# lixirui142/VidToMe

Measured on AMD Instinct MI355X. Metric: denoising steps/sec, 16-frame 512x512 SD-1.5 chunk, ratio=0.5, higher is better.
Workload: dtype f16 tokens; matching f16-MFMA filter + f32 exact refine (f32-identical indices); attention f16 MFMA with f32 accumulate

## Files before the change

### vidtome_amd/csrc/match_filter.hip

```cpp
#include "common.h"
#include "ablate.h"

#include <cstdlib>

#include <algorithm>
#include <type_traits>

namespace {

constexpr int FBD = 128;
constexpr int FBS = 256;
constexpr int FBK = 64;
constexpr int THREADS = 256;
constexpr int CAP = 64;
constexpr float SCALE = 1024.0f;
constexpr float INV_S2 = 1.0f / (1024.0f * 1024.0f);
#ifndef VTM_FILTER_PRODUCTS
#define VTM_FILTER_PRODUCTS 1
#endif
constexpr bool SRC_LO = VTM_FILTER_PRODUCTS >= 3;
constexpr bool DST_LO = VTM_FILTER_PRODUCTS >= 2;
static_assert(DST_LO || !SRC_LO, "the src lo half is only used together with the dst lo half");
constexpr float WINDOW = SRC_LO ? 6.5e-4f : DST_LO ? 1.5e-3f : 2.4e-3f;
constexpr int MAX_C = 1280;

typedef float f32x16 __attribute__((ext_vector_type(16)));
typedef _Float16 h16x8 __attribute__((ext_vector_type(8)));
typedef uint32_t u32x4 __attribute__((ext_vector_type(4)));
typedef __attribute__((address_space(3))) void lds_void;
typedef const __attribute__((address_space(1))) void glb_void;

using vtm::to_f32;

template <typename T>
__device__ __forceinline__ const T *pool_row(const T *x0, int64_t P0, const T *x1, int64_t P1, int64_t b,
                                             int64_t r, int64_t C) {
    return r < P0 ? x0 + (b * P0 + r) * C : x1 + (b * P1 + (r - P0)) * C;
}

template <typename T>
__device__ __forceinline__ void load8(const T *src, float (&f)[8]) {
    if constexpr (sizeof(T) == 4) {
        const float4 v0 = *reinterpret_cast<const float4 *>(src);
        const float4 v1 = *reinterpret_cast<const float4 *>(src + 4);
        f[0] = v0.x; f[1] = v0.y; f[2] = v0.z; f[3] = v0.w;
        f[4] = v1.x; f[5] = v1.y; f[6] = v1.z; f[7] = v1.w;
    } else {
        const uint4 v = *reinterpret_cast<const uint4 *>(src);
        const T *e = reinterpret_cast<const T *>(&v);
#pragma unroll
        for (int j = 0; j < 8; ++j) f[j] = to_f32(e[j]);
    }
}

__device__ __forceinline__ float vmax3(float a, float b, float c) {
    float d;
    asm("v_max3_f32 %0, %1, %2, %3" : "=v"(d) : "v"(a), "v"(b), "v"(c));
    return d;
}
__device__ __forceinline__ float vmax2(float a, float b) {
    float d;
    asm("v_max_f32 %0, %1, %2" : "=v"(d) : "v"(a), "v"(b));
    return d;
}

struct RowDivisor {
    float n, r1, lo;
};
__device__ __forceinline__ RowDivisor row_divisor(float n) {
    const float r = __builtin_amdgcn_rcpf(n);
    const float e = __builtin_fmaf(-n, r, 1.0f);
    return {n, __builtin_fmaf(e, r, r), fmaxf(0x1p-102f, n * 0x1p-124f)};
}
__device__ __forceinline__ bool div_ok(float x, const RowDivisor &d) { return __builtin_fabsf(x) >= d.lo || x == 0.0f; }
__device__ __forceinline__ float div_by_row(float x, const RowDivisor &d) {
    const float q = x * d.r1;
    const float t = __builtin_fmaf(-d.n, q, x);
    const float q1 = __builtin_fmaf(t, d.r1, q);
    const float t2 = __builtin_fmaf(-d.n, q1, x);
    return __builtin_fmaf(t2, d.r1, q1);
}

__device__ __forceinline__ uint32_t orderable(float f) {
    if (f != f) return 0xffffffffu;
    const uint32_t u = __float_as_uint(f + 0.0f);
    return (u & 0x80000000u) ? ~u : (u | 0x80000000u);
}
__device__ __forceinline__ float from_orderable(uint32_t o) {
    if (o == 0u) return -INFINITY;
    return __uint_as_float((o & 0x80000000u) ? (o & 0x7fffffffu) : ~o);
}

struct SplitArgs {
    const int32_t *rows;
    int64_t n;
    float *norms;
    uint4 *out_hi, *out_lo;
    int64_t n_pad;
    float *rest, *tile_rest;
    float *rest2, *tile_rest2;
};

#ifndef VTM_PREP_PIECES
#define VTM_PREP_PIECES 10
#endif
#ifndef VTM_PREP_WAVES
#define VTM_PREP_WAVES 4
#endif
constexpr int PREP_WAVES = VTM_PREP_WAVES;
constexpr int PREP_PIECES = VTM_PREP_PIECES;
constexpr int PREP_STRIDE = PREP_PIECES * 16 + 16;

template <typename T>
__global__ __launch_bounds__(64 * PREP_WAVES) void prep_operand(const T *__restrict__ x0, int64_t P0,
                                                    const T *__restrict__ x1, int64_t P1, int64_t B, int64_t C,
                                                    SplitArgs A0, SplitArgs A1, int64_t C_pad,
                                                    uint32_t *__restrict__ zero, int64_t zero_words,
                                                    unsigned long long *__restrict__ best, int64_t nbest, int64_t cut,
                                                    int64_t cut2) {
    static_assert(sizeof(T) == 2 || sizeof(T) == 4, "element size");
    static_assert(PREP_WAVES % 2 == 0, "a 128-row tile is two waves of one workgroup");
    __shared__ float wave_rest[PREP_WAVES], wave_rest2[PREP_WAVES];
    constexpr int EPP = 16 / (int)sizeof(T);
    __shared__ __attribute__((aligned(16))) char slab[PREP_WAVES][64 * PREP_STRIDE];
    const int64_t G = C_pad / 8;
    const int64_t gid = (int64_t)blockIdx.x * blockDim.x + threadIdx.x, gsz = (int64_t)gridDim.x * blockDim.x;
    for (int64_t w = gid; w < zero_words; w += gsz) zero[w] = 0u;
    for (int64_t w = gid; w < nbest; w += gsz) best[w] = 0ull;
    const int lane = threadIdx.x & 63, wave = threadIdx.x >> 6;
    char *my = slab[wave];

    int64_t idx = gid;
    const bool second = idx >= B * A0.n_pad;
    if (second) idx -= B * A0.n_pad;
    const SplitArgs &A = second ? A1 : A0;
    const int64_t n = A.n, n_pad = A.n_pad;
    const bool in_range = idx < B * n_pad;
    const int64_t i = in_range ? idx % n_pad : 0, b = in_range ? idx / n_pad : 0;
    const bool real = in_range && i < n;
    const T *src = real ? pool_row(x0, P0, x1, P1, b, A.rows[b * n + i], C) : x0;

    const int pieces = (int)(C * sizeof(T) / 16);
    const int nchunks = (pieces + PREP_PIECES - 1) / PREP_PIECES;
    uint4 stage[PREP_PIECES];
    auto issue = [&](int chunk) {
#pragma unroll
        for (int t = 0; t < PREP_PIECES; ++t) {
            const int q = lane + 64 * t, r = q / PREP_PIECES, col = q % PREP_PIECES;
            const T *rp = reinterpret_cast<const T *>(__shfl((unsigned long long)reinterpret_cast<uintptr_t>(src), r, 64));
            const int piece = chunk * PREP_PIECES + col;
            stage[t] = piece < pieces ? *reinterpret_cast<const uint4 *>(rp + (int64_t)piece * EPP) : make_uint4(0, 0, 0, 0);
        }
    };
    auto to_lds = [&]() {
#pragma unroll
        for (int t = 0; t < PREP_PIECES; ++t) {
            const int q = lane + 64 * t, r = q / PREP_PIECES, col = q % PREP_PIECES;
            *reinterpret_cast<uint4 *>(my + r * PREP_STRIDE + col * 16) = stage[t];
        }
    };
    auto my_piece = [&](int col, float (&f)[EPP]) {
        const uint4 v = *reinterpret_cast<const uint4 *>(my + lane * PREP_STRIDE + col * 16);
        const T *e = reinterpret_cast<const T *>(&v);
#pragma unroll
        for (int k = 0; k < EPP; ++k) f[k] = to_f32(e[k]);
    };

    float acc = 0.0f;
    issue(0);
    for (int c = 0; c < nchunks; ++c) {
        to_lds();
        if (c + 1 < nchunks) issue(c + 1);
        const int valid = min(PREP_PIECES, pieces - c * PREP_PIECES);
        for (int col = 0; col < valid; ++col) {
            float f[EPP];
            my_piece(col, f);
#pragma unroll
            for (int k = 0; k < EPP; ++k) acc = __builtin_fmaf(f[k], f[k], acc);
        }
    }
    const float nrm = __builtin_sqrtf(acc);
    if (real) A.norms[b * n + i] = nrm;

    const float rscale = SCALE * __builtin_amdgcn_rcpf(nrm);
    uint4 *__restrict__ out_hi = in_range ? A.out_hi + (b * G) * n_pad + i : nullptr;
    uint4 *__restrict__ out_lo = (in_range && A.out_lo) ? A.out_lo + (b * G) * n_pad + i : nullptr;
    constexpr int PPG = 8 / EPP;
    float rest = 0.0f, rest2 = 0.0f;
    issue(0);
    for (int c = 0; c < nchunks; ++c) {
        to_lds();
        if (c + 1 < nchunks) issue(c + 1);
        const int valid = min(PREP_PIECES, pieces - c * PREP_PIECES);
        for (int col = 0; col + PPG <= valid; col += PPG) {
            float f[8];
            if constexpr (PPG == 1) {
                my_piece(col, f);
            } else {
                float f0[EPP], f1[EPP];
                my_piece(col, f0);
                my_piece(col + 1, f1);
#pragma unroll
                for (int k = 0; k < EPP; ++k) { f[k] = f0[k]; f[EPP + k] = f1[k]; }
            }
            uint4 vh, vl;
            _Float16 *ph = reinterpret_cast<_Float16 *>(&vh), *pl = reinterpret_cast<_Float16 *>(&vl);
#pragma unroll
            for (int e = 0; e < 8; ++e) {
                const float sc = DST_LO ? (f[e] / nrm) * SCALE : f[e] * rscale;
                const _Float16 h = (_Float16)sc;
                ph[e] = h;
                pl[e] = (_Float16)(sc - (float)h);
            }
            if (!real) vh = vl = make_uint4(0, 0, 0, 0);
            const int64_t g = ((int64_t)c * PREP_PIECES + col) / PPG;
            if (g * 8 >= cut2) {
                float sq = 0.0f;
#pragma unroll
                for (int e = 0; e < 8; ++e) sq = __builtin_fmaf((float)ph[e], (float)ph[e], sq);
                rest2 += sq;
                if (g * 8 >= cut) rest += sq;
            }
            if (in_range) {
                out_hi[g * n_pad] = vh;
                if (out_lo) out_lo[g * n_pad] = vl;
            }
        }
    }
    if (in_range)
        for (int64_t g = C / 8; g < G; ++g) {
            out_hi[g * n_pad] = make_uint4(0, 0, 0, 0);
            if (out_lo) out_lo[g * n_pad] = make_uint4(0, 0, 0, 0);
        }
    const bool bad_row = real && !(nrm >= 0x1p-100f && nrm <= 0x1p100f);
    const float rnorm = !real ? 0.0f : bad_row ? INFINITY : __builtin_sqrtf(rest) * (1.0f + 0x1p-16f);
    if (in_range && A.rest) A.rest[b * n_pad + i] = rnorm;
    float wm = rnorm;
#pragma unroll
    for (int off = 32; off > 0; off >>= 1) wm = fmaxf(wm, __shfl_xor(wm, off, 64));
    if (lane == 0) wave_rest[wave] = wm;
    const float rnorm2 = !real ? 0.0f : bad_row ? INFINITY : __builtin_sqrtf(rest2) * (1.0f + 0x1p-16f);
    if (in_range && A.rest2) A.rest2[b * n_pad + i] = rnorm2;
    float wm2 = rnorm2;
#pragma unroll
    for (int off = 32; off > 0; off >>= 1) wm2 = fmaxf(wm2, __shfl_xor(wm2, off, 64));
    if (lane == 0) wave_rest2[wave] = wm2;
    __syncthreads();
    if (in_range && A.tile_rest && (threadIdx.x & 127) == 0)
        A.tile_rest[(b * n_pad + i) / 128] = fmaxf(wave_rest[wave], wave_rest[wave + 1]);
    if (in_range && A.tile_rest2 && (threadIdx.x & 127) == 0)
        A.tile_rest2[(b * n_pad + i) / 128] = fmaxf(wave_rest2[wave], wave_rest2[wave + 1]);
}

template <bool SCOUT>
__global__ __launch_bounds__(THREADS, 2) void filter_kernel(
    const uint4 *__restrict__ ah, const uint4 *__restrict__ al, const uint4 *__restrict__ bh,
    const uint4 *__restrict__ bl, int64_t Ns, int64_t Nd, int64_t Ns_pad, int64_t Nd_pad, int64_t C_pad, int align,
    int ns_tiles, int nd_tiles, int nsplit, int tiles_per_split, int total_src_tiles, int patch_tiles,
    unsigned int *__restrict__ amax, int *__restrict__ cnt, uint2 *__restrict__ cand, int cand_rows, int *__restrict__ flags,
    const float *__restrict__ rest_a, const float *__restrict__ rest_bt, int KP, int count_blocks,
    unsigned int *__restrict__ tilemap, int map_words) {
    __shared__ __attribute__((aligned(16))) uint4 sA[2][DST_LO ? 2 : 1][8 * FBD];

    const int tid = threadIdx.x, lane = tid & 63;
    const int wave = __builtin_amdgcn_readfirstlane(tid >> 6);
    const int l31 = lane & 31, kh = lane >> 5;

    const int xcd = blockIdx.x & 7, slot = blockIdx.x >> 3;
    const int per_group = patch_tiles * nsplit;
    const int grp = (slot / per_group) * 8 + xcd;
    const int q = slot % per_group;
    const int stg = grp * patch_tiles + q % patch_tiles;
    const int split = q / patch_tiles;
    if (stg >= total_src_tiles) return;
    const int st_ = stg % ns_tiles;
    const int bi = stg / ns_tiles;
    int jt0 = split * tiles_per_split;
    int jt1 = min(jt0 + tiles_per_split, nd_tiles);
    if (jt0 >= jt1) return;
    if constexpr (!SCOUT) {
        if (tilemap != nullptr) {
            const unsigned int *row = tilemap + (int64_t)stg * map_words;
            int lo = jt1, hi = jt0;
            for (int w = jt0 >> 5; w <= (jt1 - 1) >> 5; ++w) {
                unsigned int bits = row[w];
                if (w == (jt0 >> 5)) bits &= 0xffffffffu << (jt0 & 31);
                if (w == ((jt1 - 1) >> 5) && (jt1 & 31)) bits &= 0xffffffffu >> (32 - (jt1 & 31));
                if (bits) {
                    lo = min(lo, w * 32 + __ffs(bits) - 1);
                    hi = max(hi, w * 32 + 32 - __clz(bits));
                }
            }
            lo = __builtin_amdgcn_readfirstlane(lo);
            hi = __builtin_amdgcn_readfirstlane(hi);
            if (lo >= hi) return;
            jt0 = lo;
            jt1 = hi;
        }
    }

    const int KT = SCOUT ? KP : (int)(C_pad / FBK);
    const int64_t G = C_pad / 8;
    const int steps = (jt1 - jt0) * KT;
    int n_tested = 0, n_alive = 0;
    const uint4 *srch = ah + (int64_t)bi * G * Ns_pad, *srcl = al + (int64_t)bi * G * Ns_pad;
    const uint4 *dsth = bh + (int64_t)bi * G * Nd_pad, *dstl = bl + (int64_t)bi * G * Nd_pad;
    const int64_t srow0 = (int64_t)st_ * FBS + wave * 64;

    constexpr int NB = SRC_LO ? 4 : 2;
    const uint32_t voff_b = (uint32_t)(kh * Ns_pad + srow0 + l31) * 16u;
    const int64_t bgroup = 2 * Ns_pad;
    u32x4 rb[4][2][2];
    [[maybe_unused]] auto load_b = [&](int kt, int ks, u32x4 (&dst)[2][2]) {
        const uint4 *ph = srch + (int64_t)ABL_STREAMED(kt * 4 + ks, ks) * bgroup;
        asm volatile("global_load_dwordx4 %0, %1, %2" : "=v"(dst[0][0]) : "v"(voff_b), "s"(ph));
        asm volatile("global_load_dwordx4 %0, %1, %2 offset:512" : "=v"(dst[1][0]) : "v"(voff_b), "s"(ph));
        if constexpr (SRC_LO) {
            const uint4 *pl = srcl + (int64_t)(kt * 4 + ks) * bgroup;
            asm volatile("global_load_dwordx4 %0, %1, %2" : "=v"(dst[0][1]) : "v"(voff_b), "s"(pl));
            asm volatile("global_load_dwordx4 %0, %1, %2 offset:512" : "=v"(dst[1][1]) : "v"(voff_b), "s"(pl));
        }
    };
    auto await_b = [&](auto count_tag, u32x4 (&r)[2][2]) {
        constexpr int N = decltype(count_tag)::value;
        if constexpr (SRC_LO)
            asm volatile("s_waitcnt vmcnt(%4)" : "+v"(r[0][0]), "+v"(r[1][0]), "+v"(r[0][1]), "+v"(r[1][1]) : "n"(N));
        else
            asm volatile("s_waitcnt vmcnt(%2)" : "+v"(r[0][0]), "+v"(r[1][0]) : "n"(N));
    };
    constexpr int NPIECE = DST_LO ? 8 : 4, PG = NPIECE / 2;
    const uint4 *abase[NPIECE];
    uint32_t alds[NPIECE];
#pragma unroll
    for (int t = 0; t < NPIECE; ++t) {
// ... 275 lines not shown
            h16x8 (&fh)[4] = fa[s & 1];
            h16x8 (&fn)[4] = fa[(s + 1) & 1];
#pragma unroll
            for (int j = 0; j < 8; ++j) {
                const int sb = j >> 2, ib = j & 3;
                bool alive = true;
                if constexpr (!FIRST) alive = (live & (1u << j)) != 0u;
                if (alive) {
                    f32x16 c = acc[ib][sb];
                    if constexpr (FIRST) {
#pragma unroll
                        for (int r = 0; r < 16; ++r) c[r] = 0.0f;
                    }
                    acc[ib][sb] = __builtin_amdgcn_mfma_f32_32x32x16_f16(fh[ib], __builtin_bit_cast(h16x8, rb[s][sb][0]), c, 0, 0, 0);
                }
                __builtin_amdgcn_sched_barrier(0);
                if (j < 4) {
                    ABL_LDSREAD(if constexpr (s < 3) fn[j] = __builtin_bit_cast(h16x8, sA[buf][0][((s + 1) * 2 + kh) * FBD + j * 32 + l31]);
                                else fn[j] = __builtin_bit_cast(h16x8, sA[buf ^ 1][0][kh * FBD + j * 32 + l31]);)
                    ABL_NO_LDSREAD(fn[j] = fh[j];)
                } else if (j < 6) {
                    ABL_BLOAD(if constexpr (s < 2) load_b1(pb, s + 2, j - 4, rb[s + 2][j - 4][0]);
                              else load_b1(pbn, s - 2, j - 4, rb[s - 2][j - 4][0]);)
                } else {
                    ABL_DMA(if constexpr (s == 0) load_a_piece(pa1, buf ^ 1, j - 4);
                            if constexpr (s == 3) load_a_piece(pa2, buf, j - 6);)
                    if constexpr (s == 1)
                        asm volatile("global_load_dword %0, %1, %2 sc1" : "=v"(am[j - 6]) : "v"(voff_m[j - 6]), "s"(amax_rows));
                }
                __builtin_amdgcn_sched_barrier(0);
            }
        };
        await_b(std::integral_constant<int, ABL_AWAIT_COUNT(NB + PG)>{}, rb[0]);
        if (kt == 0) group(std::integral_constant<int, 0>{}, std::true_type{});
        else group(std::integral_constant<int, 0>{}, std::false_type{});
        group(std::integral_constant<int, 1>{}, std::false_type{});
        group(std::integral_constant<int, 2>{}, std::false_type{});
        ABL_BARRIER(asm volatile("s_waitcnt vmcnt(%0) lgkmcnt(0)" ::"n"(2 * NB + 2) : "memory"); __syncthreads();)
        group(std::integral_constant<int, 3>{}, std::false_type{});
        if (kt + 1 == KP) {
            live = prune_check(jt);
            n_tested += 8;
            n_alive += __popc(live);
            if constexpr (SCOUT) {
                if (live && lane == 0) atomicOr(&tilemap[(int64_t)stg * map_words + (jt >> 5)], 1u << (jt & 31));
            }
        }
        if constexpr (!SCOUT) {
            if (ABL_WRAP_COND(wrap && live)) collect_tile(jt, std::true_type{});
        }
        if (wrap) {
            ++jt;
            live = 0xffu;
        }
        kt = kt1;
        pb = pbn;
        pa1 = pa2;
    }
#endif
    asm volatile("s_waitcnt vmcnt(0)" ::: "memory");
    if (count_blocks && lane == 0 && n_tested) {
        if (!SCOUT && tilemap != nullptr) {
            atomicAdd(&flags[7], n_tested);
        } else {
            atomicAdd(&flags[4], n_tested);
            atomicAdd(&flags[5], n_alive);
        }
    }
    if constexpr (SCOUT) return;

#pragma unroll
    for (int sb = 0; sb < 2; ++sb) {
        const int64_t srow = srow0 + sb * 32 + l31;
        if (srow >= Ns) continue;
        float rm = runmax[sb];
        if (rm > -INFINITY) {
            const uint32_t mine = orderable(rm * INV_S2);
            const uint32_t prev = atomicMax(&amax[out_row0 + srow], mine);
            rm = fmaxf(rm, from_orderable(prev) * (SCALE * SCALE));
        }
#pragma unroll
        for (int e = 0; e < 4; ++e)
            if (cv[sb][e] >= rm - WS && cv[sb][e] > -INFINITY) push(srow, cv[sb][e], ci[sb][e]);
    }
}

template <typename T>
__global__ __launch_bounds__(256) void seed_kernel(const T *__restrict__ x0, int64_t P0, const T *__restrict__ x1, int64_t P1,
                                                   int64_t B, int64_t C, const int32_t *__restrict__ a_rows, int64_t Ns,
                                                   const int32_t *__restrict__ b_rows, int64_t Nd,
                                                   const float *__restrict__ na, const float *__restrict__ nb, int align,
                                                   int64_t seed_L, int64_t N, const int32_t *__restrict__ pos1,
                                                   const int32_t *__restrict__ table, unsigned int *__restrict__ amax, int dry,
                                                   unsigned int *__restrict__ seed_lb, float lb_margin) {
    constexpr int LPR = 8;
    const int64_t g = ((int64_t)blockIdx.x * blockDim.x + threadIdx.x) / LPR;
    const int sub = threadIdx.x & (LPR - 1);
    if (g >= B * Ns) return;
    const int64_t b = g / Ns, i = g % Ns;
    const int32_t ra = a_rows[b * Ns + i];
    int64_t pos = -1;
    if (ra < seed_L) pos = ra % N;
    else if (pos1 != nullptr && ra - P0 >= 0 && ra - P0 < P1) pos = pos1[b * P1 + (ra - P0)];
    int64_t j = -1;
    if (pos >= 0 && pos < N) j = table ? (int64_t)table[b * N + pos] : pos;
    if (j < 0 || j >= Nd) return;
    const T *pa = pool_row(x0, P0, x1, P1, b, ra, C);
    const T *pb = pool_row(x0, P0, x1, P1, b, b_rows[b * Nd + j], C);
    float acc = 0.0f;
    for (int64_t k = sub * 8; k < C; k += LPR * 8) {
        float fa[8], fb[8];
        load8(pa + k, fa);
        load8(pb + k, fb);
#pragma unroll
        for (int e = 0; e < 8; ++e) acc = __builtin_fmaf(fa[e], fb[e], acc);
    }
#pragma unroll
    for (int off = LPR / 2; off > 0; off >>= 1) acc += __shfl_xor(acc, off, 64);
    if (sub == 0) {
        const float s0 = (acc / na[b * Ns + i]) / nb[b * Nd + j];
        const float s = s0 - 1e-4f;
        const bool acc_ok = __builtin_fabsf(acc) >= 0x1p-100f || (na[b * Ns + i] >= 0x1p-40f && nb[b * Nd + j] >= 0x1p-40f);
        if (s == s && __builtin_fabsf(s) <= 1.5f && acc_ok && !dry) {
            atomicMax(&amax[align ? i : b * Ns + i], orderable(s));
            atomicMax(&seed_lb[align ? i : b * Ns + i], orderable(s0 - lb_margin));
        }
    }
}

#ifndef VTM_RROWS
#define VTM_RROWS 64
#endif
constexpr int RROWS = VTM_RROWS;
static_assert(RROWS == 32 || RROWS == 64 || RROWS == 128 || RROWS == 256, "refine rows per workgroup");
template <typename T>
__global__ __launch_bounds__(256) void refine_kernel(const T *__restrict__ x0, int64_t P0, const T *__restrict__ x1,
                                                     int64_t P1, int64_t B, int64_t C,
                                                     const int32_t *__restrict__ a_rows, int64_t Ns,
                                                     const int32_t *__restrict__ b_rows, int64_t Nd,
                                                     const float *__restrict__ na, const float *__restrict__ nb,
                                                     int align, int *__restrict__ flags, int64_t rows_out,
                                                     const unsigned int *__restrict__ amax, const int *__restrict__ cnt,
                                                     const uint2 *__restrict__ cand, int *__restrict__ ovf_cnt,
                                                     int *__restrict__ ovf_rows, uint2 *__restrict__ pairs,
                                                     const float *__restrict__ tile_rest, int64_t n_tile_rest,
                                                     unsigned long long *__restrict__ best,
                                                     const int32_t *__restrict__ src_order,
                                                     const int32_t *__restrict__ dst_order) {
    __shared__ int wave_tot[4];
    __shared__ int s_base;
    const int tid = threadIdx.x, lane = tid & 63, wave = tid >> 6;
    {
        bool bad = false;
        for (int64_t t = tid; t < n_tile_rest; t += 256) bad |= !(tile_rest[t] < INFINITY);
        if (__syncthreads_or(bad)) {
            if (blockIdx.x == 0 && tid == 0) {
                flags[0] = 1;
                flags[1] = 1;
            }
            return;
        }
    }
    const int64_t row = (int64_t)blockIdx.x * RROWS + tid;
    const bool live = tid < RROWS && row < rows_out;
    const int n = live ? cnt[row] : 0;
    const float thr = live ? from_orderable(amax[row]) - WINDOW : 0.0f;
// ... 302 lines not shown
#pragma unroll
                        for (int sb = 0; sb < XSB; ++sb) {
                            f32x16 c = acc[ib][sb];
                            if (kt == 0 && g == 0 && e == 0) {
#pragma unroll
                                for (int r = 0; r < 16; ++r) c[r] = 0.0f;
                            }
                            acc[ib][sb] = __builtin_amdgcn_mfma_f32_32x32x2f32(av, bv[sb][e], c, 0, 0, 0);
                        }
                    }
                }
            }
            if (wrap) {
                const int dst0 = jt * XD + 4 * kh;
                const bool full = (int64_t)(jt + 1) * XD <= Nd;
#pragma unroll
                for (int sb = 0; sb < XSB; ++sb) {
                    float bv_ = bestv[sb];
                    uint32_t bi_ = besti[sb];
#pragma unroll
                    for (int ib = 0; ib < 4; ++ib) {
#pragma unroll
                        for (int r = 0; r < 16; ++r) {
                            const int d = dst0 + ib * 32 + (r & 3) + 8 * (r >> 2);
                            const float sc = acc[ib][sb][r];
                            bool upd = !(sc <= bv_) && (bv_ == bv_);
                            uint32_t od = (uint32_t)d;
                            if constexpr (ORD) {
                                od = sOrd[jt & 1][d - jt * XD];
                                upd = upd || (((sc == bv_) || (sc != sc && bv_ != bv_)) && od < bi_);
                            }
                            if (!full) upd = upd && (d < Nd);
                            bv_ = upd ? sc : bv_;
                            bi_ = upd ? od : bi_;
                        }
                    }
                    bestv[sb] = bv_;
                    besti[sb] = bi_;
                }
                ++jt;
                kt = 0;
            } else if (can_prune && kt + 1 == KX) {
                const float rb = rest_bt[bi * rest_tiles + jt] * (1.0f + 0x1p-9f) * INV_S2;
                bool dead = true;
#pragma unroll
                for (int sb = 0; sb < XSB; ++sb) {
                    float pm = -INFINITY;
#pragma unroll
                    for (int ib = 0; ib < 4; ++ib)
#pragma unroll
                        for (int r = 0; r < 16; ++r) pm = fmaxf(pm, acc[ib][sb][r]);
                    dead = dead && (pm + rest_l[sb] * rb + 1e-4f < fmaxf(bestv[sb], floor_[sb]));
                }
                if (__syncthreads_and(dead)) {
                    ++jt;
                    kt = 0;
                    if (jt < jt1) {
                        dst_rows(jt);
                        fetch(0);
                    }
                } else {
                    ++kt;
                }
            } else {
                ++kt;
            }
        }
#pragma unroll
        for (int sb = 0; sb < XSB; ++sb) {
            const int64_t i = listed(wave * (32 * XSB) + sb * 32 + l31);
            if (i >= 0 && besti[sb] != 0xffffffffu) {
                const uint32_t col = besti[sb] + (align ? (uint32_t)(bi * Nd) : 0u);
                const int64_t orow = align ? (ORD ? (int64_t)src_order[i] : i) : l * Ns + (ORD ? (int64_t)src_order[l * Ns + i] : i);
                atomicMax(&best[orow], ((unsigned long long)orderable(bestv[sb]) << 32) | (uint32_t)(~col));
            }
        }
        item = next_item();
    }
}

inline size_t align_up(size_t v) { return (v + 255) & ~(size_t)255; }

struct Layout {
    size_t na, nb, ah, al, bh, bl, amax, cnt, seedlb, tilemap, cand, flags, ovf_cnt, ovf, pairs, rest_a, rest_bt, rest_a2, rest_bt2, total;
    int64_t Ns_pad, Nd_pad, C64;
};

Layout make_layout(int64_t B, int64_t C, int64_t Ns, int64_t Nd, int align) {
    Layout L;
    L.Ns_pad = vtm::cdiv(Ns, FBS) * FBS;
    L.Nd_pad = vtm::cdiv(Nd, FBS) * FBS;
    L.C64 = vtm::cdiv(C, 64) * 64;
    const int64_t rows_out = align ? Ns : B * Ns;
    size_t o = 0;
    auto take = [&](size_t bytes) { size_t at = o; o += align_up(bytes); return at; };
    L.na = take((size_t)B * Ns * 4);
    L.nb = take((size_t)B * Nd * 4);
    L.ah = take((size_t)B * L.C64 * L.Ns_pad * 2);
    L.al = take(SRC_LO ? (size_t)B * L.C64 * L.Ns_pad * 2 : 0);
    L.bh = take((size_t)B * L.C64 * L.Nd_pad * 2);
    L.bl = take(DST_LO ? (size_t)B * L.C64 * L.Nd_pad * 2 : 0);
    L.amax = take((size_t)rows_out * 4);
    L.cnt = take((size_t)rows_out * 4);
    L.seedlb = take((size_t)rows_out * 4);
    L.tilemap = take((size_t)B * (L.Ns_pad / FBS) * ((L.Nd_pad / FBD + 31) / 32) * 4);
    L.flags = take(256);
    L.ovf_cnt = take((size_t)B * 4);
    L.cand = take((size_t)rows_out * CAP * 8);
    L.ovf = take((size_t)rows_out * 4);
    L.pairs = take((size_t)rows_out * CAP * 8);
    L.rest_a = take((size_t)B * L.Ns_pad * 4);
    L.rest_bt = take((size_t)B * (L.Nd_pad / FBD) * 4);
    L.rest_a2 = take((size_t)B * L.Ns_pad * 4);
    L.rest_bt2 = take((size_t)B * (L.Nd_pad / FBD) * 4);
    L.total = o;
    return L;
}

struct DebugEnv {
    int kp5, kp, nsplit;
    bool seed_dry, nsplit_r4, no_xprune;
};
const DebugEnv &debug_env() {
    static const DebugEnv e = [] {
        auto num = [](const char *name) {
            const char *v = getenv(name);
            return v ? atoi(v) : -1;
        };
        DebugEnv d;
        d.kp5 = num("VTM_DEBUG_KP5");
        d.kp = num("VTM_DEBUG_KP");
        d.nsplit = num("VTM_DEBUG_NSPLIT");
        d.seed_dry = getenv("VTM_DEBUG_SEED_DRY") != nullptr;
        d.nsplit_r4 = getenv("VTM_DEBUG_NSPLIT_R4") != nullptr;
        d.no_xprune = getenv("VTM_DEBUG_NOXPRUNE") != nullptr;
        return d;
    }();
    return e;
}

}

VTM_EXPORT size_t vtm_match_filtered_ws_bytes(int64_t B, int64_t C, int64_t Ns, int64_t Nd, int align) {
    if (B <= 0 || C <= 0 || Ns <= 0 || Nd <= 0) return 0;
    return make_layout(B, C, Ns, Nd, align).total;
}

static int match_filtered_impl(const void *x0, int64_t P0, const void *x1, int64_t P1, int dtype, int64_t B,
                               int64_t C, const int32_t *a_rows, int64_t Ns, const int32_t *b_rows, int64_t Nd,
                               int align, void *ws, size_t ws_bytes, uint64_t *best, int32_t *flags_out,
                               int64_t seed_L, int64_t seed_N, const int32_t *seed_pos1, const int32_t *seed_table,
                               int mode, const int32_t *src_order, const int32_t *dst_order, vtm_stream_t stream) {
    VTM_REQUIRE(x0 && a_rows && b_rows && ws && best, "vtm_match_filtered: null pointer");
    const int scout_steps = (mode >> 8) & 0xff;
    mode &= 0xff;
    VTM_REQUIRE((src_order == nullptr) == (dst_order == nullptr), "vtm_match_filtered_ordered: both inverse maps or none");
    VTM_REQUIRE(mode == VTM_MATCH_ONE_LAUNCH || mode == VTM_MATCH_SCOUT_RANGE, "vtm_match_filtered: bad mode %d", mode);
    VTM_REQUIRE(B > 0 && C > 0 && C % 8 == 0 && Ns > 0 && Nd > 0, "vtm_match_filtered: bad sizes");
    VTM_REQUIRE(P1 == 0 || x1, "vtm_match_filtered: x1 is null but P1 > 0");
    VTM_REQUIRE(B * Nd < (1ll << 32) - 1, "vtm_match_filtered: index space overflow");
    VTM_REQUIRE(C <= MAX_C, "vtm_match_filtered: C=%lld > %d (error window derived for C <= %d; use vtm_match)",
                (long long)C, MAX_C, MAX_C);
    const Layout L = make_layout(B, C, Ns, Nd, align);
    if (ws_bytes < L.total)
        return vtm::fail(VTM_EWORKSPACE, "vtm_match_filtered: workspace %zu < %zu bytes", ws_bytes, L.total);
    hipStream_t s = vtm::as_stream(stream);
    char *w = static_cast<char *>(ws);
    float *na = (float *)(w + L.na), *nb = (float *)(w + L.nb);
    uint4 *ah = (uint4 *)(w + L.ah), *al = (uint4 *)(w + L.al), *bh = (uint4 *)(w + L.bh), *bl = (uint4 *)(w + L.bl);
    unsigned int *amax = (unsigned int *)(w + L.amax);
    int *cnt = (int *)(w + L.cnt), *flags = (int *)(w + L.flags);
    uint2 *cand = (uint2 *)(w + L.cand);
    int *ovf_rows = (int *)(w + L.ovf), *ovf_cnt = (int *)(w + L.ovf_cnt);
    uint2 *pairs = (uint2 *)(w + L.pairs);
    const int64_t rows_out = align ? Ns : B * Ns;
    VTM_REQUIRE(rows_out * CAP < (1ll << 31), "vtm_match_filtered: too many rows for the 32-bit candidate index");

    VTM_REQUIRE(dtype == VTM_F32 || dtype == VTM_F16 || dtype == VTM_BF16, "vtm_match_filtered: bad dtype");
    const int KT = (int)(L.C64 / FBK);
    int KP = (VTM_FILTER_PRODUCTS == 1 && KT >= 4) ? (2 * KT + 2) / 5 : 0;
    const DebugEnv &dbg = debug_env();
    if (VTM_FILTER_PRODUCTS == 1 && KT == 5 && dbg.kp5 >= 0 && dbg.kp5 < KT) KP = dbg.kp5;
    if (VTM_FILTER_PRODUCTS == 1 && dbg.kp >= 0 && dbg.kp < KT) KP = dbg.kp;
    const bool prune = KP > 0 && KP < KT;
    float *rest_a = (float *)(w + L.rest_a), *rest_bt = (float *)(w + L.rest_bt);
    const int64_t cut = prune ? (int64_t)KP * FBK : L.C64;
    const int KPS = (prune && mode == VTM_MATCH_SCOUT_RANGE && scout_steps > 0 && scout_steps < KP) ? scout_steps : KP;
    float *rest_a2 = (float *)(w + L.rest_a2), *rest_bt2 = (float *)(w + L.rest_bt2);
    const int64_t cut2 = KPS < KP ? (int64_t)KPS * FBK : cut;
    {
        const SplitArgs A0{a_rows, Ns, na, ah, SRC_LO ? al : nullptr, L.Ns_pad, rest_a, nullptr, KPS < KP ? rest_a2 : nullptr, nullptr};
        const SplitArgs A1{b_rows, Nd, nb, bh, DST_LO ? bl : nullptr, L.Nd_pad, nullptr, rest_bt, nullptr, KPS < KP ? rest_bt2 : nullptr};
        const int64_t total = B * (L.Ns_pad + L.Nd_pad);
        unsigned long long *bp0 = reinterpret_cast<unsigned long long *>(best);
        uint32_t *zp = reinterpret_cast<uint32_t *>(w + L.amax);
        const int64_t zw = (int64_t)((L.cand - L.amax) / 4);
        const dim3 grid((unsigned)vtm::cdiv(total, 64 * PREP_WAVES)), block(64 * PREP_WAVES);
        switch (dtype) {
            case VTM_F32:
                hipLaunchKernelGGL(prep_operand<float>, grid, block, 0, s, (const float *)x0, P0, (const float *)x1, P1,
                                   B, C, A0, A1, L.C64, zp, zw, bp0, rows_out, cut, cut2);
                break;
            case VTM_F16:
                hipLaunchKernelGGL(prep_operand<__half>, grid, block, 0, s, (const __half *)x0, P0, (const __half *)x1,
                                   P1, B, C, A0, A1, L.C64, zp, zw, bp0, rows_out, cut, cut2);
                break;
            default:
                hipLaunchKernelGGL(prep_operand<vtm_bf16>, grid, block, 0, s, (const vtm_bf16 *)x0, P0,
                                   (const vtm_bf16 *)x1, P1, B, C, A0, A1, L.C64, zp, zw, bp0, rows_out, cut, cut2);
        }
    }

    if (seed_N > 0) {
        const int dry = dbg.seed_dry;
        unsigned int *seedlb = (unsigned int *)(w + L.seedlb);
        const float lb_margin = (4.0f * (float)C + 32.0f) * 0x1p-24f + 1e-6f;
        const dim3 grid((unsigned)vtm::cdiv(B * Ns * 8, 256)), block(256);
        switch (dtype) {
            case VTM_F32:
                hipLaunchKernelGGL(seed_kernel<float>, grid, block, 0, s, (const float *)x0, P0, (const float *)x1, P1, B, C, a_rows,
                                   Ns, b_rows, Nd, (const float *)na, (const float *)nb, align, seed_L, seed_N, seed_pos1, seed_table, amax, dry, seedlb, lb_margin);
                break;
            case VTM_F16:
                hipLaunchKernelGGL(seed_kernel<__half>, grid, block, 0, s, (const __half *)x0, P0, (const __half *)x1, P1, B, C,
                                   a_rows, Ns, b_rows, Nd, (const float *)na, (const float *)nb, align, seed_L, seed_N, seed_pos1, seed_table, amax, dry, seedlb, lb_margin);
                break;
            default:
                hipLaunchKernelGGL(seed_kernel<vtm_bf16>, grid, block, 0, s, (const vtm_bf16 *)x0, P0, (const vtm_bf16 *)x1, P1, B,
                                   C, a_rows, Ns, b_rows, Nd, (const float *)na, (const float *)nb, align, seed_L, seed_N, seed_pos1, seed_table, amax, dry, seedlb, lb_margin);
        }
    }
    {
        const int ns_tiles = (int)(L.Ns_pad / FBS), nd_tiles = (int)(L.Nd_pad / FBD);
        const int total_src_tiles = (int)(B * ns_tiles);
        const int max_patch = (int64_t)16 * FBS * L.C64 * 2 <= (3 << 20) ? 16 : 8;
        const int tiles_per_xcd = (int)vtm::cdiv(total_src_tiles, 8);
        const int patches_per_xcd = (int)vtm::cdiv(tiles_per_xcd, max_patch);
        const int patch_tiles = (int)vtm::cdiv(tiles_per_xcd, patches_per_xcd);
        const int ngroups = (int)vtm::cdiv(total_src_tiles, patch_tiles);
        auto wgs_per_xcd = [&](int ns) {
            const int tps = (int)vtm::cdiv(nd_tiles, ns);
            return patches_per_xcd * patch_tiles * (int)vtm::cdiv(nd_tiles, tps);
        };
        int nsplit;
        if (dbg.nsplit_r4) {
            int64_t want = vtm::cdiv(1536, (int64_t)ns_tiles * B);
            nsplit = (int)(want < 1 ? 1 : want);
            if (nd_tiles >= 32) nsplit = 8;
            if (nsplit > nd_tiles / 4) nsplit = nd_tiles / 4 > 0 ? nd_tiles / 4 : 1;
            if (nsplit > 8) nsplit = 8;
            if (nsplit == 8) {
                const int slots = vtm::device_cus() / 8 * 2;
                for (int ns = 7; ns >= 6; --ns)
                    if (wgs_per_xcd(8) > slots && wgs_per_xcd(ns) <= slots) {
                        nsplit = ns;
                        break;
                    }
            }
        } else {
            const int slots = vtm::device_cus() / 8 * 2;
            double best_cost = 1e30;
            nsplit = 1;
            for (int ns = 1; ns <= 16 && ns <= nd_tiles; ++ns) {
                const int tps = (int)vtm::cdiv(nd_tiles, ns);
                if ((int)vtm::cdiv(nd_tiles, tps) != ns) continue;
                if (tps < 4 && ns > 1) continue;
                const int wgs = wgs_per_xcd(ns);
                const double rounds = (wgs <= slots && wgs > slots - slots / 16) ? 2.0 : (double)vtm::cdiv(wgs, slots);
                const double cost = rounds * (tps + 1.5) + 0.25 * ns;
                if (cost < best_cost - 1e-9) {
                    best_cost = cost;
                    nsplit = ns;
                }
            }
        }
        if (dbg.nsplit >= 1 && dbg.nsplit <= 16 && dbg.nsplit <= nd_tiles) nsplit = dbg.nsplit;
        const int tiles_per_split = (int)vtm::cdiv(nd_tiles, nsplit);
        nsplit = (int)vtm::cdiv(nd_tiles, tiles_per_split);
        const int64_t grid = (int64_t)8 * vtm::cdiv(ngroups, 8) * patch_tiles * nsplit;
        const int64_t c_run = L.C64;
        const int map_words = (nd_tiles + 31) / 32;
        unsigned int *tilemap = (unsigned int *)(w + L.tilemap);
        const bool ordered = src_order != nullptr;
        const bool range_plan = mode == VTM_MATCH_SCOUT_RANGE && prune && c_run == L.C64 &&
                                (ordered ? seed_N > 0 && nd_tiles >= 2 : seed_N >= 2 * FBD && seed_N % FBD == 0);
        if (range_plan) {
            hipLaunchKernelGGL(filter_kernel<true>, dim3((unsigned)grid), dim3(THREADS), 0, s, ah, al, bh, bl, Ns, Nd, L.Ns_pad,
                               L.Nd_pad, L.C64, align, ns_tiles, nd_tiles, nsplit, tiles_per_split, total_src_tiles, patch_tiles,
                               amax, cnt, cand, (int)rows_out, flags, (const float *)(KPS < KP ? rest_a2 : rest_a),
                               (const float *)(KPS < KP ? rest_bt2 : rest_bt), KPS, flags_out != nullptr ? 1 : 0, tilemap, map_words);
            const int tps_r = ordered ? tiles_per_split : (int)(seed_N / FBD);
            const int nsplit_r = (int)vtm::cdiv(nd_tiles, tps_r);
            const int64_t grid_r = (int64_t)8 * vtm::cdiv(ngroups, 8) * patch_tiles * nsplit_r;
            hipLaunchKernelGGL(filter_kernel<false>, dim3((unsigned)grid_r), dim3(THREADS), 0, s, ah, al, bh, bl, Ns, Nd,
                               L.Ns_pad, L.Nd_pad, L.C64, align, ns_tiles, nd_tiles, nsplit_r, tps_r, total_src_tiles, patch_tiles,
                               amax, cnt, cand, (int)rows_out, flags, (const float *)rest_a, (const float *)rest_bt, KP,
                               flags_out != nullptr ? 1 : 0, tilemap, map_words);
        } else {
            hipLaunchKernelGGL(filter_kernel<false>, dim3((unsigned)grid), dim3(THREADS), 0, s, ah, al, bh, bl, Ns, Nd, L.Ns_pad,
                               L.Nd_pad, c_run, align, ns_tiles, nd_tiles, nsplit, tiles_per_split, total_src_tiles, patch_tiles,
                               amax, cnt, cand, (int)rows_out, flags, prune ? (const float *)rest_a : nullptr,
                               prune ? (const float *)rest_bt : nullptr, prune ? KP : 0x7fffffff, flags_out != nullptr ? 1 : 0,
                               (unsigned int *)nullptr, map_words);
        }
    }
    bool flags_direct = false;
    {
        const dim3 grid((unsigned)vtm::cdiv(rows_out, RROWS)), block(256);
        unsigned long long *bp = reinterpret_cast<unsigned long long *>(best);
        const int64_t n_tile_rest = B * (L.Nd_pad / FBD);
#define VTM_REFINE_ARGS a_rows, Ns, b_rows, Nd, na, nb, align, flags, rows_out, amax, cnt, cand, ovf_cnt, ovf_rows, pairs, \
                        (const float *)rest_bt, n_tile_rest, bp, src_order, dst_order
        const int xd_tiles = (int)vtm::cdiv(Nd, XD);
        int xsplit = xd_tiles / 8;
        xsplit = xsplit < 1 ? 1 : xsplit > 16 ? 16 : xsplit;
        const int xtps = (int)vtm::cdiv(xd_tiles, xsplit);
        xsplit = (int)vtm::cdiv(xd_tiles, xtps);
        const dim3 xgrid((unsigned)((XS == 128 ? 2 : 1) * vtm::device_cus()));
        const int KX = dbg.no_xprune ? 0 : (int)(cut / XK);
        int32_t *flags_pub = nullptr;
        if (flags_out) {
            hipPointerAttribute_t attr;
            if (hipPointerGetAttributes(&attr, flags_out) == hipSuccess &&
                (attr.type == hipMemoryTypeDevice || attr.type == hipMemoryTypeHost || attr.type == hipMemoryTypeManaged))
                flags_pub = attr.type == hipMemoryTypeHost && attr.devicePointer ? (int32_t *)attr.devicePointer : flags_out;
            else
                (void)hipGetLastError();
        }
        flags_direct = flags_pub != nullptr;
#define VTM_XPRUNE_ARGS (const float *)rest_a, (const float *)rest_bt, KX, L.Ns_pad, L.Nd_pad / FBD, (const unsigned int *)(w + L.seedlb), \
                        flags + 6, src_order, dst_order, flags_pub
        switch (dtype) {
            case VTM_F32:
                hipLaunchKernelGGL(refine_kernel<float>, grid, block, 0, s, (const float *)x0, P0, (const float *)x1, P1,
                                   B, C, VTM_REFINE_ARGS);
                hipLaunchKernelGGL((src_order ? exact_rows_kernel<float, true> : exact_rows_kernel<float, false>), xgrid, block, 0, s, (const float *)x0, P0, (const float *)x1, P1,
                                   B, C, a_rows, Ns, b_rows, Nd, na, nb, align, flags, ovf_cnt, ovf_rows, bp, xsplit, xtps, VTM_XPRUNE_ARGS);
                break;
            case VTM_F16:
                hipLaunchKernelGGL(refine_kernel<__half>, grid, block, 0, s, (const __half *)x0, P0, (const __half *)x1,
                                   P1, B, C, VTM_REFINE_ARGS);
                hipLaunchKernelGGL((src_order ? exact_rows_kernel<__half, true> : exact_rows_kernel<__half, false>), xgrid, block, 0, s, (const __half *)x0, P0, (const __half *)x1,
                                   P1, B, C, a_rows, Ns, b_rows, Nd, na, nb, align, flags, ovf_cnt, ovf_rows, bp, xsplit, xtps, VTM_XPRUNE_ARGS);
                break;
            default:
                hipLaunchKernelGGL(refine_kernel<vtm_bf16>, grid, block, 0, s, (const vtm_bf16 *)x0, P0,
                                   (const vtm_bf16 *)x1, P1, B, C, VTM_REFINE_ARGS);
                hipLaunchKernelGGL((src_order ? exact_rows_kernel<vtm_bf16, true> : exact_rows_kernel<vtm_bf16, false>), xgrid, block, 0, s, (const vtm_bf16 *)x0, P0,
                                   (const vtm_bf16 *)x1, P1, B, C, a_rows, Ns, b_rows, Nd, na, nb, align, flags, ovf_cnt,
                                   ovf_rows, bp, xsplit, xtps, VTM_XPRUNE_ARGS);
        }
    }
    if (int rc = vtm::launch_status("vtm_match_filtered")) return rc;

    if (flags_out && !flags_direct) {
        const hipError_t e = hipMemcpyAsync(flags_out, flags, 8 * sizeof(int), hipMemcpyDefault, s);
        if (e != hipSuccess) return vtm::fail(VTM_ELAUNCH, "vtm_match_filtered: copy: %s", hipGetErrorString(e));
    }
    return VTM_OK;
}

VTM_EXPORT int vtm_match_filtered(const void *x0, int64_t P0, const void *x1, int64_t P1, int dtype, int64_t B,
                                  int64_t C, const int32_t *a_rows, int64_t Ns, const int32_t *b_rows, int64_t Nd,
                                  int align, void *ws, size_t ws_bytes, uint64_t *best, int32_t *flags_out,
                                  vtm_stream_t stream) {
    return match_filtered_impl(x0, P0, x1, P1, dtype, B, C, a_rows, Ns, b_rows, Nd, align, ws, ws_bytes, best, flags_out, 0, 0,
                               nullptr, nullptr, VTM_MATCH_ONE_LAUNCH, nullptr, nullptr, stream);
}

VTM_EXPORT int vtm_match_filtered_seeded(const void *x0, int64_t P0, const void *x1, int64_t P1, int dtype, int64_t B,
                                         int64_t C, const int32_t *a_rows, int64_t Ns, const int32_t *b_rows, int64_t Nd,
                                         int align, void *ws, size_t ws_bytes, uint64_t *best, int32_t *flags_out,
                                         int64_t seed_L, int64_t seed_N, const int32_t *seed_pos1, const int32_t *seed_table,
// ... 31 lines not shown
```

Before: 21.85.

## Add int8 MFMA scout pass with rigorous quantization error bounds for tile pruning

When the scout prefix is 64 or 128 channels, the prep kernel now also quantizes the leading f16 channels to int8, using a per-row step for sources and a per-tile step for destinations, and records L1 norms. A new scout kernel runs i8 32x32x32 MFMA on these int8 operands and marks destination tiles whose bound, widened by a quantization-error slack, can still reach the threshold. This replaces the f16 scout filter with cheaper, higher-throughput integer math. In exchange it adds quantization work and extra workspace to prep, and the looser bound may keep more tiles alive for the refine pass.

```diff
diff --git a/vidtome_amd/csrc/match_filter.hip b/vidtome_amd/csrc/match_filter.hip
--- a/vidtome_amd/csrc/match_filter.hip
+++ b/vidtome_amd/csrc/match_filter.hip
@@ -99,6 +99,9 @@
     int64_t n_pad;
     float *rest, *tile_rest;
     float *rest2, *tile_rest2;
+    uint4 *out_q;
+    float *q_step, *q_l1;
+    bool q_tile;
 };
 
 #ifndef VTM_PREP_PIECES
@@ -117,10 +120,10 @@
                                                     SplitArgs A0, SplitArgs A1, int64_t C_pad,
                                                     uint32_t *__restrict__ zero, int64_t zero_words,
                                                     unsigned long long *__restrict__ best, int64_t nbest, int64_t cut,
-                                                    int64_t cut2) {
+                                                    int64_t cut2, int64_t cutq) {
     static_assert(sizeof(T) == 2 || sizeof(T) == 4, "element size");
     static_assert(PREP_WAVES % 2 == 0, "a 128-row tile is two waves of one workgroup");
-    __shared__ float wave_rest[PREP_WAVES], wave_rest2[PREP_WAVES];
+    __shared__ float wave_rest[PREP_WAVES], wave_rest2[PREP_WAVES], wave_qmax[PREP_WAVES], wave_ql1[PREP_WAVES];
     constexpr int EPP = 16 / (int)sizeof(T);
     __shared__ __attribute__((aligned(16))) char slab[PREP_WAVES][64 * PREP_STRIDE];
     const int64_t G = C_pad / 8;
@@ -187,6 +190,7 @@
     uint4 *__restrict__ out_lo = (in_range && A.out_lo) ? A.out_lo + (b * G) * n_pad + i : nullptr;
     constexpr int PPG = 8 / EPP;
     float rest = 0.0f, rest2 = 0.0f;
+    float qmax = 0.0f, ql1 = 0.0f;
     issue(0);
     for (int c = 0; c < nchunks; ++c) {
         to_lds();
@@ -214,6 +218,14 @@
             }
             if (!real) vh = vl = make_uint4(0, 0, 0, 0);
             const int64_t g = ((int64_t)c * PREP_PIECES + col) / PPG;
+            if (g * 8 < cutq) {
+#pragma unroll
+                for (int e = 0; e < 8; ++e) {
+                    const float a = __builtin_fabsf((float)ph[e]);
+                    qmax = fmaxf(qmax, a);
+                    ql1 += a;
+                }
+            }
             if (g * 8 >= cut2) {
                 float sq = 0.0f;
 #pragma unroll
@@ -250,6 +262,51 @@
         A.tile_rest[(b * n_pad + i) / 128] = fmaxf(wave_rest[wave], wave_rest[wave + 1]);
     if (in_range && A.tile_rest2 && (threadIdx.x & 127) == 0)
         A.tile_rest2[(b * n_pad + i) / 128] = fmaxf(wave_rest2[wave], wave_rest2[wave + 1]);
+
+    if (A.out_q != nullptr) {
+        float m = qmax, l1 = ql1 * (1.0f + 0x1p-16f);
+        if (A.q_tile) {
+            float wq = m, wl = l1;
+#pragma unroll
+            for (int off = 32; off > 0; off >>= 1) {
+                wq = fmaxf(wq, __shfl_xor(wq, off, 64));
+                wl = fmaxf(wl, __shfl_xor(wl, off, 64));
+            }
+            if (lane == 0) {
+                wave_qmax[wave] = wq;
+                wave_ql1[wave] = wl;
+            }
+            __syncthreads();
+            const int w0 = wave & ~1;
+            m = fmaxf(wave_qmax[w0], wave_qmax[w0 + 1]);
+            l1 = fmaxf(wave_ql1[w0], wave_ql1[w0 + 1]);
+        }
+        const float step = m * (1.0f / 127.0f) * (1.0f + 0x1p-22f);
+        if (in_range) {
+            const int64_t GQ = cutq / 16;
+            uint4 *out_q = A.out_q + (b * GQ) * n_pad + i;
+            for (int64_t gq = 0; gq < GQ; ++gq) {
+                uint4 v[2] = {out_hi[(2 * gq) * n_pad], out_hi[(2 * gq + 1) * n_pad]};
+                const _Float16 *h = reinterpret_cast<const _Float16 *>(v);
+                uint32_t w4[4] = {0u, 0u, 0u, 0u};
+#pragma unroll
+                for (int e = 0; e < 16; ++e) {
+                    const float x = (float)h[e];
+                    float qf = step > 0.0f && x == x ? __builtin_rintf(x / step) : 0.0f;
+                    qf = fminf(fmaxf(qf, -127.0f), 127.0f);
+                    w4[e >> 2] |= ((uint32_t)(int32_t)qf & 0xffu) << (8 * (e & 3));
+                }
+                out_q[gq * n_pad] = make_uint4(w4[0], w4[1], w4[2], w4[3]);
+            }
+            if (!A.q_tile) {
+                A.q_step[b * n_pad + i] = step;
+                A.q_l1[b * n_pad + i] = l1;
+            } else if ((threadIdx.x & 127) == 0) {
+                A.q_step[(b * n_pad + i) / 128] = step;
+                A.q_l1[(b * n_pad + i) / 128] = l1;
+            }
+        }
+    }
 }
 
 template <bool SCOUT>
@@ -691,6 +748,126 @@
 #pragma unroll
         for (int e = 0; e < 4; ++e)
             if (cv[sb][e] >= rm - WS && cv[sb][e] > -INFINITY) push(srow, cv[sb][e], ci[sb][e]);
+    }
+}
+
+typedef int32_t i32x4 __attribute__((ext_vector_type(4)));
+typedef int32_t i32x16 __attribute__((ext_vector_type(16)));
+constexpr float QC = 0.5f + 0x1p-15f;
+constexpr int QMAX_K = 128;
+
+template <int NK>
+__global__ __launch_bounds__(THREADS, 2) void scout_q_kernel(
+    const uint4 *__restrict__ aq, const uint4 *__restrict__ bq, const float *__restrict__ qs_a, const float *__restrict__ ql1_a,
+    const float *__restrict__ qs_bt, const float *__restrict__ ql1_bt, int64_t Ns, int64_t Ns_pad, int64_t Nd_pad, float acc_slack,
+    int align, int ns_tiles, int nd_tiles, int nsplit, int tiles_per_split, int total_src_tiles, int patch_tiles,
+    const unsigned int *__restrict__ amax, int *__restrict__ flags, const float *__restrict__ rest_a,
+    const float *__restrict__ rest_bt, int count_blocks, unsigned int *__restrict__ tilemap, int map_words) {
+    static_assert(NK == 2 || NK == 4, "one or two 64-channel steps");
+    constexpr int GQ = NK * 2;
+    constexpr int K = NK * 32;
+    __shared__ __attribute__((aligned(16))) uint4 sQ[2][GQ * FBD];
+
+    const int tid = threadIdx.x, lane = tid & 63;
+    const int wave = __builtin_amdgcn_readfirstlane(tid >> 6);
+    const int l31 = lane & 31, kh = lane >> 5;
+    const int xcd = blockIdx.x & 7, slot = blockIdx.x >> 3;
+    const int per_group = patch_tiles * nsplit;
+    const int grp = (slot / per_group) * 8 + xcd;
+    const int q = slot % per_group;
+    const int stg = grp * patch_tiles + q % patch_tiles;
+    const int split = q / patch_tiles;
+    if (stg >= total_src_tiles) return;
+    const int st_ = stg % ns_tiles;
+    const int bi = stg / ns_tiles;
+    const int jt0 = split * tiles_per_split;
+    const int jt1 = min(jt0 + tiles_per_split, nd_tiles);
+    if (jt0 >= jt1) return;
+
+    const int64_t srow0 = (int64_t)st_ * FBS + wave * 64;
+    const int64_t out_row0 = align ? 0 : (int64_t)bi * Ns;
+    const uint4 *const dst_base = bq + (int64_t)bi * GQ * Nd_pad;
+    auto load_tile = [&](int jt, int buf) {
+#pragma unroll
+        for (int t = 0; t < NK; ++t) {
+            const int p = (wave * NK + t) >> 1, half = (wave * NK + t) & 1;
+            const uint4 *g = dst_base + (int64_t)p * Nd_pad + (int64_t)jt * FBD + half * 64;
+            const uint32_t lds_off = (uint32_t)reinterpret_cast<uintptr_t>((lds_void *)&sQ[buf][p * FBD + half * 64]);
+            asm volatile("s_mov_b32 m0, %0\n\ts_nop 0\n\tglobal_load_lds_dwordx4 %1, %2"
+                         :
+                         : "s"(lds_off), "v"((uint32_t)lane * 16u), "s"(g)
+                         : "memory");
+        }
+    };
+    load_tile(jt0, 0);
+    i32x4 fb[NK][2];
+    float da[2], l1a[2], need[2], rest_l[2];
+#pragma unroll
+    for (int sb = 0; sb < 2; ++sb) {
+        const int64_t srow = srow0 + sb * 32 + l31;
+#pragma unroll
+        for (int ks = 0; ks < NK; ++ks)
+            fb[ks][sb] = __builtin_bit_cast(i32x4, aq[((int64_t)bi * GQ + 2 * ks + kh) * Ns_pad + srow]);
+        need[sb] = srow < Ns ? from_orderable(amax[out_row0 + srow]) * (SCALE * SCALE) - WINDOW * SCALE * SCALE : INFINITY;
+        da[sb] = qs_a[(int64_t)bi * Ns_pad + srow];
+        l1a[sb] = ql1_a[(int64_t)bi * Ns_pad + srow];
+        rest_l[sb] = rest_a[(int64_t)bi * Ns_pad + srow];
+    }
+    asm volatile("s_waitcnt vmcnt(0)" : "+v"(fb[0][0]), "+v"(fb[0][1]), "+v"(fb[1][0]), "+v"(fb[1][1]) : : "memory");
+    if constexpr (NK == 4) asm volatile("" : "+v"(fb[2][0]), "+v"(fb[2][1]), "+v"(fb[3][0]), "+v"(fb[3][1]));
+    __syncthreads();
+
+    int n_tested = 0, n_alive = 0;
+    for (int jt = jt0; jt < jt1; ++jt) {
+        const int buf = (jt - jt0) & 1;
+        if (jt + 1 < jt1) load_tile(jt + 1, buf ^ 1);
+        i32x16 acc[4][2];
+#pragma unroll
+        for (int ks = 0; ks < NK; ++ks) {
+            i32x4 fa[4];
+#pragma unroll
+            for (int ib = 0; ib < 4; ++ib) fa[ib] = __builtin_bit_cast(i32x4, sQ[buf][(2 * ks + kh) * FBD + ib * 32 + l31]);
+#pragma unroll
+            for (int sb = 0; sb < 2; ++sb)
+#pragma unroll
+                for (int ib = 0; ib < 4; ++ib) {
+                    i32x16 c;
+                    if (ks == 0) {
+#pragma unroll
+                        for (int r = 0; r < 16; ++r) c[r] = 0;
+                    } else {
+                        c = acc[ib][sb];
+                    }
+                    acc[ib][sb] = __builtin_amdgcn_mfma_i32_32x32x32_i8(fa[ib], fb[ks][sb], c, 0, 0, 0);
+                }
+        }
+        const float dt = qs_bt[(int64_t)bi * nd_tiles + jt], l1t = ql1_bt[(int64_t)bi * nd_tiles + jt];
+        const float rb = rest_bt[(int64_t)bi * nd_tiles + jt];
+        uint32_t mask = 0;
+#pragma unroll
+        for (int sb = 0; sb < 2; ++sb) {
+            const float dd = da[sb] * dt;
+            const float slack = (QC * (da[sb] * l1t + dt * l1a[sb]) + (float)K * QC * QC * dd) * (1.0f + 0x1p-20f) + acc_slack;
+            const float thr = need[sb] - rest_l[sb] * rb - slack;
+#pragma unroll
+            for (int ib = 0; ib < 4; ++ib) {
+                const i32x16 &v = acc[ib][sb];
+                int m = v[0];
+#pragma unroll
+                for (int r = 1; r < 16; ++r) m = max(m, v[r]);
+                const float p = (float)m * dd;
+                if (__any(p + __builtin_fabsf(p) * 0x1p-20f >= thr)) mask |= 1u << (sb * 4 + ib);
+            }
+        }
+        n_tested += 8;
+        n_alive += __popc(mask);
+        if (mask && lane == 0) atomicOr(&tilemap[(int64_t)stg * map_words + (jt >> 5)], 1u << (jt & 31));
+        asm volatile("s_waitcnt vmcnt(0)" ::: "memory");
+        __syncthreads();
+    }
+    if (count_blocks && lane == 0 && n_tested) {
+        atomicAdd(&flags[4], n_tested);
+        atomicAdd(&flags[5], n_alive);
     }
 }
 
@@ -1159,7 +1336,8 @@
 inline size_t align_up(size_t v) { return (v + 255) & ~(size_t)255; }
 
 struct Layout {
-    size_t na, nb, ah, al, bh, bl, amax, cnt, seedlb, tilemap, cand, flags, ovf_cnt, ovf, pairs, rest_a, rest_bt, rest_a2, rest_bt2, total;
+    size_t na, nb, ah, al, bh, bl, amax, cnt, seedlb, tilemap, cand, flags, ovf_cnt, ovf, pairs, rest_a, rest_bt, rest_a2, rest_bt2,
+        aq, bq, qs_a, ql1_a, qs_bt, ql1_bt, total;
     int64_t Ns_pad, Nd_pad, C64;
 };
 
@@ -1190,6 +1368,12 @@
     L.rest_bt = take((size_t)B * (L.Nd_pad / FBD) * 4);
     L.rest_a2 = take((size_t)B * L.Ns_pad * 4);
     L.rest_bt2 = take((size_t)B * (L.Nd_pad / FBD) * 4);
+    L.aq = take((size_t)B * L.Ns_pad * QMAX_K);
+    L.bq = take((size_t)B * L.Nd_pad * QMAX_K);
+    L.qs_a = take((size_t)B * L.Ns_pad * 4);
+    L.ql1_a = take((size_t)B * L.Ns_pad * 4);
+    L.qs_bt = take((size_t)B * (L.Nd_pad / FBD) * 4);
+    L.ql1_bt = take((size_t)B * (L.Nd_pad / FBD) * 4);
     L.total = o;
     return L;
 }
@@ -1265,9 +1449,19 @@
     const int KPS = (prune && mode == VTM_MATCH_SCOUT_RANGE && scout_steps > 0 && scout_steps < KP) ? scout_steps : KP;
     float *rest_a2 = (float *)(w + L.rest_a2), *rest_bt2 = (float *)(w + L.rest_bt2);
     const int64_t cut2 = KPS < KP ? (int64_t)KPS * FBK : cut;
+    const bool ordered = src_order != nullptr;
+    const int nd_tiles = (int)(L.Nd_pad / FBD);
+    const bool range_plan = mode == VTM_MATCH_SCOUT_RANGE && prune &&
+                            (ordered ? seed_N > 0 && nd_tiles >= 2 : seed_N >= 2 * FBD && seed_N % FBD == 0);
+    const int64_t cutq = range_plan && KPS * FBK <= QMAX_K ? (int64_t)KPS * FBK : 0;
+    uint4 *aq = (uint4 *)(w + L.aq), *bq = (uint4 *)(w + L.bq);
+    float *qs_a = (float *)(w + L.qs_a), *ql1_a = (float *)(w + L.ql1_a);
+    float *qs_bt = (float *)(w + L.qs_bt), *ql1_bt = (float *)(w + L.ql1_bt);
     {
-        const SplitArgs A0{a_rows, Ns, na, ah, SRC_LO ? al : nullptr, L.Ns_pad, rest_a, nullptr, KPS < KP ? rest_a2 : nullptr, nullptr};
-        const SplitArgs A1{b_rows, Nd, nb, bh, DST_LO ? bl : nullptr, L.Nd_pad, nullptr, rest_bt, nullptr, KPS < KP ? rest_bt2 : nullptr};
+        const SplitArgs A0{a_rows, Ns, na, ah, SRC_LO ? al : nullptr, L.Ns_pad, rest_a, nullptr, KPS < KP ? rest_a2 : nullptr, nullptr,
+                           cutq ? aq : nullptr, qs_a, ql1_a, false};
+        const SplitArgs A1{b_rows, Nd, nb, bh, DST_LO ? bl : nullptr, L.Nd_pad, nullptr, rest_bt, nullptr, KPS < KP ? rest_bt2 : nullptr,
+                           cutq ? bq : nullptr, qs_bt, ql1_bt, true};
         const int64_t total = B * (L.Ns_pad + L.Nd_pad);
         unsigned long long *bp0 = reinterpret_cast<unsigned long long *>(best);
         uint32_t *zp = reinterpret_cast<uint32_t *>(w + L.amax);
@@ -1276,15 +1470,15 @@
         switch (dtype) {
             case VTM_F32:
                 hipLaunchKernelGGL(prep_operand<float>, grid, block, 0, s, (const float *)x0, P0, (const float *)x1, P1,
-                                   B, C, A0, A1, L.C64, zp, zw, bp0, rows_out, cut, cut2);
+                                   B, C, A0, A1, L.C64, zp, zw, bp0, rows_out, cut, cut2, cutq);
                 break;
             case VTM_F16:
                 hipLaunchKernelGGL(prep_operand<__half>, grid, block, 0, s, (const __half *)x0, P0, (const __half *)x1,
-                                   P1, B, C, A0, A1, L.C64, zp, zw, bp0, rows_out, cut, cut2);
+                                   P1, B, C, A0, A1, L.C64, zp, zw, bp0, rows_out, cut, cut2, cutq);
                 break;
             default:
                 hipLaunchKernelGGL(prep_operand<vtm_bf16>, grid, block, 0, s, (const vtm_bf16 *)x0, P0,
-                                   (const vtm_bf16 *)x1, P1, B, C, A0, A1, L.C64, zp, zw, bp0, rows_out, cut, cut2);
+                                   (const vtm_bf16 *)x1, P1, B, C, A0, A1, L.C64, zp, zw, bp0, rows_out, cut, cut2, cutq);
         }
     }
 
@@ -1308,7 +1502,7 @@
         }
     }
     {
-        const int ns_tiles = (int)(L.Ns_pad / FBS), nd_tiles = (int)(L.Nd_pad / FBD);
+        const int ns_tiles = (int)(L.Ns_pad / FBS);
         const int total_src_tiles = (int)(B * ns_tiles);
         const int max_patch = (int64_t)16 * FBS * L.C64 * 2 <= (3 << 20) ? 16 : 8;
         const int tiles_per_xcd = (int)vtm::cdiv(total_src_tiles, 8);
@@ -1358,14 +1552,20 @@
         const int64_t c_run = L.C64;
         const int map_words = (nd_tiles + 31) / 32;
         unsigned int *tilemap = (unsigned int *)(w + L.tilemap);
-        const bool ordered = src_order != nullptr;
-        const bool range_plan = mode == VTM_MATCH_SCOUT_RANGE && prune && c_run == L.C64 &&
-                                (ordered ? seed_N > 0 && nd_tiles >= 2 : seed_N >= 2 * FBD && seed_N % FBD == 0);
-        if (range_plan) {
-            hipLaunchKernelGGL(filter_kernel<true>, dim3((unsigned)grid), dim3(THREADS), 0, s, ah, al, bh, bl, Ns, Nd, L.Ns_pad,
-                               L.Nd_pad, L.C64, align, ns_tiles, nd_tiles, nsplit, tiles_per_split, total_src_tiles, patch_tiles,
-                               amax, cnt, cand, (int)rows_out, flags, (const float *)(KPS < KP ? rest_a2 : rest_a),
-                               (const float *)(KPS < KP ? rest_bt2 : rest_bt), KPS, flags_out != nullptr ? 1 : 0, tilemap, map_words);
+        if (range_plan && c_run == L.C64) {
+            const float *rest_s = KPS < KP ? rest_a2 : rest_a, *rest_st = KPS < KP ? rest_bt2 : rest_bt;
+            const float acc_slack = (float)(C + 8) * 0x1p-23f * SCALE * SCALE;
+            if (cutq == 64 || cutq == 128) {
+                auto kq = cutq == 64 ? scout_q_kernel<2> : scout_q_kernel<4>;
+                hipLaunchKernelGGL(kq, dim3((unsigned)grid), dim3(THREADS), 0, s, aq, bq, qs_a, ql1_a, qs_bt, ql1_bt, Ns, L.Ns_pad,
+                                   L.Nd_pad, acc_slack, align, ns_tiles, nd_tiles, nsplit, tiles_per_split, total_src_tiles,
+                                   patch_tiles, amax, flags, rest_s, rest_st, flags_out != nullptr ? 1 : 0, tilemap, map_words);
+            } else {
+                hipLaunchKernelGGL(filter_kernel<true>, dim3((unsigned)grid), dim3(THREADS), 0, s, ah, al, bh, bl, Ns, Nd, L.Ns_pad,
+                                   L.Nd_pad, L.C64, align, ns_tiles, nd_tiles, nsplit, tiles_per_split, total_src_tiles, patch_tiles,
+                                   amax, cnt, cand, (int)rows_out, flags, rest_s, rest_st, KPS, flags_out != nullptr ? 1 : 0,
+                                   tilemap, map_words);
+            }
             const int tps_r = ordered ? tiles_per_split : (int)(seed_N / FBD);
             const int nsplit_r = (int)vtm::cdiv(nd_tiles, tps_r);
             const int64_t grid_r = (int64_t)8 * vtm::cdiv(ngroups, 8) * patch_tiles * nsplit_r;
```

After: 22.16, median of 6. 1.01x the previous value.
